# yisol/IDM-VTON

Measured on AMD Instinct MI355X. Metric: try-on images/sec at 768x1024, 30 DDIM steps, guidance 2.0, higher is better.
Workload: dtype bf16; 1 GPU; BASELINE.json configs[1]: 768x1024, 30 steps, batch 2/GPU, guidance 2.0, bf16 storage / fp32 accumulate, scheduler ddim, hipGraph on, GarmentNet batched over 6 timesteps, GarmentNet(block b+1)||TryonNet(block b) two-stream overlap on; images_per_call=2, parallelism=dp1 (image shards, one start-up RCCL weight broadcast), rccl_ranks=1

## Files before the change

### idm-vton_amd/csrc/attention.hip

```cpp
#include "common.cuh"

struct AttnParams {
    int B, heads, Nq;
    const void* q; int ldq; uint32_t qbytes;
    void* out; int ldo;
    int nseg;
    const void* k[2]; int ldk[2]; uint32_t kbytes[2];
    const void* vt[2]; int ldvt[2]; uint32_t vtbytes[2];
    int nk[2]; int krows[2]; int seg_b0[2];
    float ip_scale;
    int nqb, chunk, parts;
    int pp_flags; float pp_thr;
    int q_prescaled;
    int seg_nb[2];
    const int32_t* seg_ix[2];
    const int32_t* seg_nkt[2];
};

#define NEG_BIG (-1.0e30f)


__device__ __forceinline__ bool attn_work(const AttnParams& p, int bid, int& b, int& h, int& qb) {
    const int x = bid & 7, j = bid >> 3;
    const int u = j / p.chunk, r = j - u * p.chunk;
// ... 727 lines not shown
#pragma unroll
            for (int r = 0; r < 16; ++r) {
                const float pv = __builtin_amdgcn_exp2f(sacc[kb][r]);
                if constexpr (!LSUM) { if (r & 1) ps1 += pv; else ps0 += pv; }
                pf[kb * 2 + (r >> 3)][r & 7] = (T)pv;
            }
        if constexpr (!LSUM) l_run += ps0 + ps1;
        __builtin_amdgcn_sched_barrier(0);
        DBG_STAMP(5);
        const float nm = -m_run;
#pragma unroll
        for (int r = 0; r < 16; ++r) { sacc[0][r] = nm; sacc[1][r] = nm; }
        __builtin_amdgcn_sched_barrier(0);
        DBG_STAMP(6);
    };
    auto phase_barrier = [&]() {
        __builtin_amdgcn_sched_barrier(0);
        __builtin_amdgcn_s_barrier();
        __builtin_amdgcn_sched_barrier(0);
        asm volatile("" ::: "memory");
    };
    auto mid_barrier = [&](int s) {
        __builtin_amdgcn_sched_barrier(0);
        if (s + 2 <= sf.nt) asm volatile("s_waitcnt vmcnt(%0) lgkmcnt(0)" ::"n"(IPW) : "memory");
        else asm volatile("s_waitcnt vmcnt(0) lgkmcnt(0)" ::: "memory");
        __builtin_amdgcn_s_barrier();
        __builtin_amdgcn_sched_barrier(0);
        asm volatile("" ::: "memory");
    };
    int b0i = 0, b1i = 1;
    auto rotate = [&]() { b0i = b1i; b1i = b1i + 1 == ST ? 0 : b1i + 1; };

#ifdef ATTN_DBG
    dbg_t = __builtin_readcyclecounter();
#endif
    if (grp == 0) {
        read_frags(smem);
        for (int s = 0; s <= sf.nt; ++s) {
            asm volatile("s_waitcnt lgkmcnt(0)" ::: "memory");
            DBG_STAMP(2);
            phase_barrier();
            DBG_STAMP(3);
            mfma_block();
            __builtin_amdgcn_sched_barrier(0);
            DBG_STAMP(0);
            mid_barrier(s);
            DBG_STAMP(1);
            if ((ABL != 2 && ABL < 5) && s + 1 <= sf.nt) read_frags(smem + b1i * 16384);
            __builtin_amdgcn_sched_barrier(0);
            if ((ABL != 1 && ABL < 5) && s + 3 <= sf.nt) issue_stage(s + 3, b0i);
            if (s < sf.nt) valu_block(s);
            rotate();
        }
    } else {
        for (int s = 0; s <= sf.nt; ++s) {
            DBG_STAMP(2);
            phase_barrier();
            DBG_STAMP(3);
            if (ABL != 2 && ABL < 5) read_frags(smem + b0i * 16384);
            __builtin_amdgcn_sched_barrier(0);
            if (s >= 1) valu_block(s - 1);
            __builtin_amdgcn_sched_barrier(0);
            DBG_STAMP(0);
            mid_barrier(s);
            DBG_STAMP(1);
            mfma_block();
            __builtin_amdgcn_sched_barrier(0);
            if ((ABL != 1 && ABL < 5) && s + 3 <= sf.nt) issue_stage(s + 3, b0i);
            rotate();
        }
    }
#ifdef ATTN_DBG
    if (lane == 0 && blockIdx.x < 4096) {
#pragma unroll
        for (int i = 0; i < 8; ++i) g_attn_dbg[(blockIdx.x * 8 + wave) * 8 + i] = dbg_acc[i];
    }
#endif

    const float lt = LSUM ? lacc[0] : xhalf_sum(l_run);
    const float inv = lt > 0.f ? 1.0f / lt : 0.f;
    finalise_store<T>(p, b, h, q_row, u, oacc, inv);
}

template <typename T, int NW, int ABL = 0>
__global__ __launch_bounds__(NW * 64, 2) void attn_sp_kernel(const AttnParams p) {
    typedef typename VT<T>::v8 v8;
    constexpr int QB = 32 * NW, IPW = 16 / NW, ST = 3;
    __shared__ __attribute__((aligned(1024))) char smem[ST * 16384 + NW * 4096];

    const int lane = threadIdx.x & 63;
    const int wave = uniform(threadIdx.x >> 6);
    const int u = lane >> 5, l31 = lane & 31;
    const float limit = p.pp_thr;

    int b, h, qb;
    if (!sp_work(p, blockIdx.x, b, h, qb)) return;
    const int q_row = qb * QB + wave * 32 + l31;

    stage_q_tile(make_rsrc(p.q, p.qbytes), p.Nq, p.ldq, smem + ST * 16384 + wave * 4096, b, h, qb * QB + wave * 32, lane);
    SegFacts sf;
    seg_facts(p, b, sf);

    const int lrow = lane >> 3, lslot = lane & 7;
    const bool is_k = wave < NW / 2;
    uint32_t rb[IPW];
    auto seg_base = [&](int sg) {
        const size_t bsg = (size_t)(sg ? sf.bsg1 : sf.bsg0);
#pragma unroll
        for (int i = 0; i < IPW; ++i) {
            const int R = ((wave * IPW + i) & 7) * 8 + lrow;
            const int c = lslot ^ ((R >> 1) & 7);
            rb[i] = is_k ? (uint32_t)(((bsg * p.krows[sg] + R) * p.ldk[sg] + h * 64 + c * 8) * 2)
                         : (uint32_t)(((bsg * p.heads * 64 + h * 64 + R) * p.ldvt[sg] + c * 8) * 2);
        }
    };
    auto lane_lim = [&](int i) {
        const int R = ((wave * IPW + i) & 7) * 8 + lrow;
        const int c = lslot ^ ((R >> 1) & 7);
        return is_k ? R : 16 * (c >> 1) + 4 * (c & 1);
    };
    const uint32_t tstep0 = is_k ? (uint32_t)(64 * p.ldk[0] * 2) : 128u, tstep1 = is_k ? (uint32_t)(64 * p.ldk[1] * 2) : 128u;
    const __amdgpu_buffer_rsrc_t rs0 = is_k ? make_rsrc(p.k[0], p.kbytes[0]) : make_rsrc(p.vt[0], p.vtbytes[0]);
    const __amdgpu_buffer_rsrc_t rs1 = is_k ? make_rsrc(p.k[1], p.kbytes[1]) : make_rsrc(p.vt[1], p.vtbytes[1]);
    int ld_t = is_k ? 0 : -2, ld_room = sf.nt0 > 0 ? sf.nk0 : sf.nk1;
    bool ld_seg1 = sf.nt0 == 0;
    uint32_t ld_off = 0;
    seg_base(ld_seg1 ? 1 : 0);
    auto issue_next = [&](int bufi) {
        char* dst = smem + bufi * 16384 + wave * (IPW * 1024);
        if (ld_t < 0 || ld_t >= sf.nt) {
#pragma unroll
            for (int i = 0; i < IPW; ++i) dma16(rs0, dst + i * 1024, OOB_SENTINEL);
        } else {
            if (!ld_seg1 && ld_t == sf.nt0) { ld_seg1 = true; ld_off = 0; ld_room = sf.nk1; seg_base(1); }
            if (ld_room >= 64) {
#pragma unroll
                for (int i = 0; i < IPW; ++i) { if (ld_seg1) dma16(rs1, dst + i * 1024, rb[i] + ld_off); else dma16(rs0, dst + i * 1024, rb[i] + ld_off); }
            } else {
#pragma unroll
                for (int i = 0; i < IPW; ++i) {
                    const uint32_t off = lane_lim(i) < ld_room ? rb[i] + ld_off : OOB_SENTINEL;
                    if (ld_seg1) dma16(rs1, dst + i * 1024, off); else dma16(rs0, dst + i * 1024, off);
                }
            }
            ld_off += ld_seg1 ? tstep1 : tstep0;
            ld_room -= 64;
        }
        ++ld_t;
    };

    int f_addr[2], f_swz[2];
#pragma unroll
    for (int kb = 0; kb < 2; ++kb) { const int r = kb * 32 + l31; f_addr[kb] = r * 128; f_swz[kb] = (r >> 1) & 7; }

    f32x16 oacc[2], sA[2], sB[2];
    v8 P[4];
#pragma unroll
    for (int db = 0; db < 2; ++db)
#pragma unroll
        for (int r = 0; r < 16; ++r) { oacc[db][r] = 0.f; sA[db][r] = 0.f; sB[db][r] = 0.f; }
#pragma unroll
    for (int ks = 0; ks < 4; ++ks)
#pragma unroll
        for (int j = 0; j < 8; ++j) P[ks][j] = (T)0.f;
    float m_run = 0.f, l_run = 0.f;
    float lim_cur = -1.f, floor_cur = -3.0e38f;
    {
        const int nz = absent_keys(p, sf);
        if (nz > 0) { l_run = u == 0 ? (float)nz : 0.f; lim_cur = limit; floor_cur = 0.f; }
    }

    const int last = sf.nt + 1;
    issue_next(0);
    issue_next(1);
    wait_vmcnt<IPW>();
    __builtin_amdgcn_s_barrier();
    __builtin_amdgcn_sched_barrier(0);
    asm volatile("" ::: "memory");
    const char* const dq = smem + ST * 16384 + wave * 4096 + l31 * 128;
    v8 qf[4];
#pragma unroll
    for (int s4 = 0; s4 < 4; ++s4) qf[s4] = *(const v8*)(dq + (((2 * s4 + u) ^ ((l31 >> 1) & 7)) << 4));

    auto k_frag = [&](const char* buf, int kb, int s4) { return *(const v8*)(buf + f_addr[kb] + (((2 * s4 + u) ^ f_swz[kb]) << 4)); };
    auto v_frag = [&](const char* buf, int db, int ks) { return *(const v8*)(buf + 8192 + f_addr[db] + (((2 * ks + u) ^ f_swz[db]) << 4)); };

    int cbuf = 0, ibuf = 2;
    auto sync_stage = [&](int i) -> const char* {
        if (i + 1 <= last) wait_vmcnt<IPW>(); else wait_vmcnt<0>();
        if constexpr (!(ABL & 16)) __builtin_amdgcn_s_barrier();
        __builtin_amdgcn_sched_barrier(0);
        asm volatile("" ::: "memory");
        if (!(ABL & 8) && i + 2 <= last) issue_next(ibuf);
        const char* buf = smem + cbuf * 16384;
        cbuf = cbuf + 1 == ST ? 0 : cbuf + 1;
        ibuf = ibuf + 1 == ST ? 0 : ibuf + 1;
        return buf;
    };

    auto block = [&](int jvalid, const char* buf, f32x16 (&Scur)[2], f32x16 (&Snext)[2], float (&ps)[4]) {
        if (jvalid < 64) {
#pragma unroll
            for (int kb = 0; kb < 2; ++kb)
#pragma unroll
                for (int r = 0; r < 16; ++r) {
                    const int key = kb * 32 + (r & 3) + 8 * (r >> 2) + 4 * u;
                    if (key >= jvalid) Scur[kb][r] = NEG_BIG;
                }
        }
        __builtin_amdgcn_sched_barrier(0);
        v8 vf[2][4], kf[2][4];
#pragma unroll
        for (int ks = 0; ks < 4; ++ks) {
            if constexpr (ABL & 4) { vf[0][ks] = qf[ks]; vf[1][ks] = qf[ks]; kf[0][ks] = qf[ks]; kf[1][ks] = qf[ks]; }
            else { vf[0][ks] = v_frag(buf, 0, ks); vf[1][ks] = v_frag(buf, 1, ks); kf[0][ks] = k_frag(buf, 0, ks); kf[1][ks] = k_frag(buf, 1, ks); }
        }
        if constexpr (!(ABL & 2)) {
#pragma unroll
            for (int ks = 0; ks < 4; ++ks) {
                oacc[0] = VT<T>::mfma(vf[0][ks], P[ks], oacc[0]);
                oacc[1] = VT<T>::mfma(vf[1][ks], P[ks], oacc[1]);
                Snext[0] = VT<T>::mfma(kf[0][ks], qf[ks], Snext[0]);
                Snext[1] = VT<T>::mfma(kf[1][ks], qf[ks], Snext[1]);
            }
        } else {
#pragma unroll
            for (int ks = 0; ks < 4; ++ks) asm volatile("" :: "v"(vf[0][ks]), "v"(vf[1][ks]), "v"(kf[0][ks]), "v"(kf[1][ks]), "v"(P[ks]));
        }
        ps[0] = ps[1] = ps[2] = ps[3] = 0.f;
#pragma unroll
        for (int kb = 0; kb < 2; ++kb)
#pragma unroll
            for (int r = 0; r < 16; ++r) {
                const float pv = (ABL & 1) ? Scur[kb][r] : __builtin_amdgcn_exp2f(Scur[kb][r]);
                ps[r & 3] += pv;
                P[kb * 2 + (r >> 3)][r & 7] = (T)pv;
            }
#pragma unroll
        for (int ks = 0; ks < 4; ++ks) asm volatile("" : "+v"(P[ks]));
        __builtin_amdgcn_sched_barrier(0);
    };
    auto tail = [&](f32x16 (&Scur)[2], f32x16 (&Snext)[2], float (&ps)[4]) {
        float psum = (ps[0] + ps[1]) + (ps[2] + ps[3]);
        if (__any(!(psum <= lim_cur))) {
            float mx = fmaxf(Scur[0][0], Scur[1][0]);
#pragma unroll
            for (int r = 1; r < 16; ++r) mx = fmaxf(fmaxf(mx, Scur[0][r]), Scur[1][r]);
            mx = xhalf_max(mx);
            const float delta = fmaxf(mx, floor_cur);
            const float alpha = __builtin_amdgcn_exp2f(fminf(-delta, 0.f));
            l_run *= alpha;
#pragma unroll
            for (int db = 0; db < 2; ++db)
#pragma unroll
                for (int r = 0; r < 16; ++r) oacc[db][r] *= alpha;
            m_run += delta;
            lim_cur = limit; floor_cur = 0.f;
            float q0 = 0.f, q1 = 0.f;
#pragma unroll
            for (int kb = 0; kb < 2; ++kb)
#pragma unroll
                for (int r = 0; r < 16; ++r) {
                    const float pv = __builtin_amdgcn_exp2f(Scur[kb][r] - delta);
                    if (r & 1) q1 += pv; else q0 += pv;
                    P[kb * 2 + (r >> 3)][r & 7] = (T)pv;
                    Snext[kb][r] -= delta;
                }
            psum = q0 + q1;
        }
        l_run += psum;
        const float nm = -m_run;
#pragma unroll
        for (int r = 0; r < 16; ++r) { Scur[0][r] = nm; Scur[1][r] = nm; }
        __builtin_amdgcn_sched_barrier(0);
    };

    {
        const char* buf = sync_stage(0);
#pragma unroll
        for (int ks = 0; ks < 4; ++ks) {
            sA[0] = VT<T>::mfma(k_frag(buf, 0, ks), qf[ks], sA[0]);
            sA[1] = VT<T>::mfma(k_frag(buf, 1, ks), qf[ks], sA[1]);
        }
        __builtin_amdgcn_sched_barrier(0);
    }
    float ps[4];
    int i = 1, jv = sf.nt0 > 0 ? sf.nk0 : sf.nk1;
    auto next_valid = [&](int ii) { jv -= 64; if (ii == sf.nt0 && sf.nt1 > 0) jv = sf.nk1; };
    for (; i + 1 <= sf.nt; i += 2) {
        const char* buf = sync_stage(i);
        block(jv, buf, sA, sB, ps);
        tail(sA, sB, ps);
        next_valid(i);
        buf = sync_stage(i + 1);
        block(jv, buf, sB, sA, ps);
        tail(sB, sA, ps);
        next_valid(i + 1);
    }
    if (i <= sf.nt) {
        const char* buf = sync_stage(i);
        block(jv, buf, sA, sB, ps);
        tail(sA, sB, ps);
    }
    if (sf.nt > 0) {
        const char* buf = sync_stage(sf.nt + 1);
#pragma unroll
        for (int ks = 0; ks < 4; ++ks) {
            oacc[0] = VT<T>::mfma(v_frag(buf, 0, ks), P[ks], oacc[0]);
            oacc[1] = VT<T>::mfma(v_frag(buf, 1, ks), P[ks], oacc[1]);
        }
    }
    const float lt = xhalf_sum(l_run);
    const float inv = lt > 0.f ? 1.0f / lt : 0.f;
    finalise_store<T>(p, b, h, q_row, u, oacc, inv);
}

template <typename T, int MODE>
static int launch_attn(AttnParams& p, int tune, hipStream_t st) {
    const long bh = (long)p.B * p.heads;
    int nw = 4, stg = 3;
    if (bh * ((p.Nq + 255) / 256) >= 200) { nw = 8; stg = 2; }
    else if (bh * ((p.Nq + 127) / 128) < 64 && p.Nq <= 64) { nw = 2; stg = 2; }
    if (tune) { nw = tune & 0xff; stg = (tune >> 8) & 0xff; }
    else if (MODE == IDMVTON_ATTN_SELF && p.q_prescaled && p.Nq >= 128) {
        nw = (bh * ((p.Nq + 255) / 256) >= 400 && p.Nq >= 2048) ? 8 : 4; stg = 3;
        tune = (16 << 16) | (3 << 8) | nw;
    } else if (MODE == IDMVTON_ATTN_SELF && bh * ((p.Nq + 255) / 256) >= 200 && p.Nq >= 1024) {
        tune = (2 << 16) | (2 << 8) | 8; nw = 8; stg = 2;
    }
    const int kern = (tune >> 16) & 0xff, flags = (tune >> 24) & 3, sel = (tune >> 26) & 3;
    static const float thr_tab[4] = {4.f, 0.f, 8.f, 2.f};
    typedef void (*kernel_t)(const AttnParams);
    auto launch = [&](kernel_t k, bool sp, int qrows) -> int {
        dim3 grid;
        if (sp) sp_grid(p, qrows, grid); else attn_grid(p, qrows, grid);
        hipLaunchKernelGGL(k, grid, dim3(qrows * 2), 0, st, p);
        CHECK_LAUNCH("attn_fwd");
        return IDMVTON_OK;
    };
    if (kern == 2 || kern == 3) {
        const bool deep = kern == 3 && p.q_prescaled;
        if (MODE != IDMVTON_ATTN_SELF || nw != 8 || (stg != 2 && stg != 3))
            return idmvton_set_error(IDMVTON_E_ARG, "attn_fwd: the ping-pong kernel needs SELF mode, 8 waves, 2 or 3 stages");
        p.pp_flags = flags;
        p.pp_thr = thr_tab[sel];
        return launch(!deep ? attn_pp_kernel<T, 2, false> : stg == 2 ? attn_pp_kernel<T, 2, true> : attn_pp_kernel<T, 3, true>, false, 256);
    }
    if (kern >= 4 && kern <= 6) {
        p.pp_flags = 0; p.pp_thr = 4.f;
        if (MODE != IDMVTON_ATTN_SELF) return idmvton_set_error(IDMVTON_E_ARG, "attn_fwd: ablation kernels are SELF mode only");
        if (nw != 8 || stg != 2)
            return idmvton_set_error(IDMVTON_E_ARG, "attn_fwd: the ablation kernels are 8 waves, 2 stages (tune waves=%d stages=%d)", nw, stg);
        return launch(kern == 4 ? attn_pp_kernel<T, 2, false, 1> : kern == 5 ? attn_pp_kernel<T, 2, false, 2> : attn_pp_kernel<T, 2, false, 3>, false, 256);
    }
    if (kern == 7 || kern == 8) {
        if (MODE != IDMVTON_ATTN_SELF || !p.q_prescaled)
            return idmvton_set_error(IDMVTON_E_ARG, "attn_fwd: the prefetch kernel needs SELF mode and a pre-multiplied q");
        if (nw != 8 || stg != 3)
            return idmvton_set_error(IDMVTON_E_ARG, "attn_fwd: the prefetch kernel is 8 waves, 3 stages (tune waves=%d stages=%d)", nw, stg);
        p.pp_flags = 0;
        p.pp_thr = thr_tab[sel];
        return launch(kern == 7 ? attn_pf_kernel<T, true> : attn_pf_kernel<T, false>, false, 256);
    }
    if (kern == 16) {
        if (MODE != IDMVTON_ATTN_SELF || !p.q_prescaled)
            return idmvton_set_error(IDMVTON_E_ARG, "attn_fwd: the software-pipelined kernel needs SELF mode and a pre-multiplied q");
        if ((nw != 4 && nw != 8) || stg != 3)
            return idmvton_set_error(IDMVTON_E_ARG, "attn_fwd: the software-pipelined kernel is 4 or 8 waves, 3 stages (tune waves=%d stages=%d)", nw, stg);
        static const float lim_tab[4] = {512.f, 32.f, 8192.f, 128.f};
        p.pp_thr = lim_tab[sel];
        return nw == 4 ? launch(attn_sp_kernel<T, 4>, true, 128) : launch(attn_sp_kernel<T, 8>, true, 256);
    }
#ifdef ATTN_DBG
    if (kern >= 32 && kern < 160) {
        p.pp_flags = 0; p.pp_thr = 512.f;
        switch (kern - 32) {
#define SPA(m) case m: return launch(attn_sp_kernel<T, 8, m>, true, 256);
        SPA(0) SPA(1) SPA(2) SPA(3) SPA(4) SPA(8) SPA(12) SPA(15) SPA(16) SPA(31) SPA(29)
#undef SPA
        default: return idmvton_set_error(IDMVTON_E_ARG, "attn_fwd: ablation mask not built");
        }
    }
    if (kern >= 9 && kern <= 14) {
        p.pp_flags = 0; p.pp_thr = 4.f;
        switch (kern) {
        case 9: return launch(attn_pf_kernel<T, true, 1>, false, 256);
        case 10: return launch(attn_pf_kernel<T, true, 2>, false, 256);
        case 11: return launch(attn_pf_kernel<T, true, 3>, false, 256);
        case 12: return launch(attn_pf_kernel<T, true, 4>, false, 256);
        case 13: return launch(attn_pf_kernel<T, true, 5>, false, 256);
        default: return launch(attn_pf_kernel<T, true, 6>, false, 256);
        }
    }
#endif
    if (kern) return idmvton_set_error(IDMVTON_E_ARG, "attn_fwd: unknown kernel selector in tune");
    kernel_t k = nullptr;
#define ATTN_CASE(NW_, ST_) if (nw == NW_ && stg == ST_) k = attn_kernel<T, MODE, NW_, ST_>;
    ATTN_CASE(2, 2) ATTN_CASE(4, 2) ATTN_CASE(8, 2)
    ATTN_CASE(2, 3) ATTN_CASE(4, 3) ATTN_CASE(8, 3)
    ATTN_CASE(2, 4) ATTN_CASE(4, 4) ATTN_CASE(8, 4)
#undef ATTN_CASE
    if (!k) return idmvton_set_error(IDMVTON_E_ARG, "attn_fwd: unsupported tune (waves=%d stages=%d)", nw, stg);
    return launch(k, false, 32 * nw);
}

static int attn_fwd_impl(const idmvton_attn_args* a, const int32_t* seg_nb, const int32_t* const* seg_index, const int32_t* const* seg_nk, void* stream) {
    CHECK_ARG(a != nullptr, IDMVTON_E_ARG, "attn_fwd: null args");
    CHECK_ARG(a->dtype == IDMVTON_F16 || a->dtype == IDMVTON_BF16, IDMVTON_E_DTYPE, "attn_fwd: dtype %d", a->dtype);
    CHECK_ARG(a->mode == IDMVTON_ATTN_SELF || a->mode == IDMVTON_ATTN_CROSS, IDMVTON_E_ARG, "attn_fwd: mode %d", a->mode);
    CHECK_ARG(a->B > 0 && a->heads > 0 && a->Nq > 0, IDMVTON_E_SHAPE, "attn_fwd: B=%d heads=%d Nq=%d", a->B, a->heads, a->Nq);
    CHECK_ARG(a->nseg >= 1 && a->nseg <= 2, IDMVTON_E_SHAPE, "attn_fwd: nseg=%d", a->nseg);
    if (a->mode == IDMVTON_ATTN_CROSS) CHECK_ARG(a->nseg == 2 && a->seg_b0[0] == 0 && a->seg_b0[1] == 0, IDMVTON_E_ARG,
                                                 "attn_fwd: CROSS needs two segments present for every batch");
    CHECK_ARG(a->q && a->out && a->ldq % 8 == 0 && a->ldo % 8 == 0 && ((uintptr_t)a->q & 15) == 0 && ((uintptr_t)a->out & 15) == 0,
              IDMVTON_E_ALIGN, "attn_fwd: q/out alignment (ldq=%d ldo=%d)", a->ldq, a->ldo);
    CHECK_ARG(a->ldq >= a->heads * 64 && a->ldo >= a->heads * 64, IDMVTON_E_SHAPE, "attn_fwd: ldq/ldo < heads*64");
    AttnParams p;
    p.B = a->B; p.heads = a->heads; p.Nq = a->Nq; p.q = a->q; p.ldq = a->ldq; p.out = a->out; p.ldo = a->ldo;
    p.nseg = a->nseg; p.ip_scale = a->ip_scale; p.nqb = 0; p.chunk = p.parts = 1; p.pp_flags = 0; p.pp_thr = 4.f; p.q_prescaled = a->q_prescaled ? 1 : 0;
    const uint64_t qb = ((uint64_t)a->B * a->Nq - 1) * a->ldq * 2 + (uint64_t)a->heads * 128;
    CHECK_ARG(qb < 0x80000000ull, IDMVTON_E_SHAPE, "attn_fwd: Q >= 2 GiB");
    p.qbytes = (uint32_t)qb;
    for (int s = 0; s < 2; ++s) {
        const int ss = s < a->nseg ? s : 0;
        CHECK_ARG(a->k[ss] && a->vt[ss] && a->nk[ss] > 0 && a->seg_b0[ss] >= 0 && a->seg_b0[ss] <= a->B,
                  IDMVTON_E_SHAPE, "attn_fwd: seg %d nk=%d b0=%d", ss, a->nk[ss], a->seg_b0[ss]);
        const int32_t* ix = seg_index ? seg_index[ss] : nullptr;
        if (ix) {
            CHECK_ARG(a->mode != IDMVTON_ATTN_CROSS, IDMVTON_E_ARG, "attn_fwd_indexed: CROSS mode takes no table (seg %d)", ss);
            CHECK_ARG(seg_nb[ss] >= 1 && a->seg_b0[ss] < a->B, IDMVTON_E_SHAPE,
                      "attn_fwd_indexed: seg %d has a table: needs seg_nb >= 1 (%d) and seg_b0 < B (%d, %d)", ss, seg_nb[ss], a->seg_b0[ss], a->B);
            CHECK_ARG(((uintptr_t)ix & 3) == 0, IDMVTON_E_ALIGN, "attn_fwd_indexed: seg %d table is not 4-byte aligned", ss);
        } else
        CHECK_ARG(seg_nb[ss] >= 0 && seg_nb[ss] <= a->B - a->seg_b0[ss], IDMVTON_E_SHAPE,
                  "attn_fwd_shared: seg %d seg_nb=%d outside [0, B - seg_b0 = %d]", ss, seg_nb[ss], a->B - a->seg_b0[ss]);
        const int32_t* nkt = seg_nk && s < a->nseg ? seg_nk[s] : nullptr;
        if (nkt) {
            CHECK_ARG(a->mode != IDMVTON_ATTN_CROSS, IDMVTON_E_ARG, "attn_fwd_ragged: CROSS mode takes no table (seg %d)", ss);
            CHECK_ARG(((uintptr_t)nkt & 3) == 0, IDMVTON_E_ALIGN, "attn_fwd_ragged: seg %d key-count table is not 4-byte aligned", ss);
        }
        CHECK_ARG(a->mode != IDMVTON_ATTN_CROSS || seg_nb[ss] == 0, IDMVTON_E_ARG, "attn_fwd_shared: CROSS mode takes seg_nb = {0, 0} (seg %d: %d)", ss, seg_nb[ss]);
        const int krows = a->k_rows[ss] > 0 ? a->k_rows[ss] : a->nk[ss];
        CHECK_ARG(krows >= a->nk[ss], IDMVTON_E_SHAPE, "attn_fwd: seg %d k_rows=%d < nk", ss, krows);
        CHECK_ARG(a->ldk[ss] % 8 == 0 && a->ldvt[ss] % 16 == 0 && a->ldvt[ss] >= ((a->nk[ss] + 15) & ~15) && a->ldk[ss] >= a->heads * 64 &&
                  ((uintptr_t)a->k[ss] & 15) == 0 && ((uintptr_t)a->vt[ss] & 15) == 0, IDMVTON_E_ALIGN,
                  "attn_fwd: seg %d ldk=%d ldvt=%d (V^T is read in key order: ldvt %% 16 == 0, ldvt >= roundup16(nk))", ss, a->ldk[ss], a->ldvt[ss]);
        const int nb = seg_nb[ss] > 0 ? seg_nb[ss] : a->B - a->seg_b0[ss];
        const uint64_t kb = (uint64_t)nb * krows * a->ldk[ss] * 2, vb = (uint64_t)nb * a->heads * 64 * a->ldvt[ss] * 2;
        CHECK_ARG(kb < 0x80000000ull && vb < 0x80000000ull, IDMVTON_E_SHAPE, "attn_fwd: seg %d K/V^T >= 2 GiB", ss);
        p.k[s] = a->k[ss]; p.ldk[s] = a->ldk[ss]; p.kbytes[s] = (uint32_t)kb;
        p.vt[s] = a->vt[ss]; p.ldvt[s] = a->ldvt[ss]; p.vtbytes[s] = (uint32_t)vb;
        p.nk[s] = a->nk[ss]; p.krows[s] = krows; p.seg_b0[s] = a->seg_b0[ss]; p.seg_nb[s] = seg_nb[ss]; p.seg_ix[s] = ix; p.seg_nkt[s] = nkt;
    }
    hipStream_t st = (hipStream_t)stream;
    if (a->dtype == IDMVTON_BF16)
        return a->mode == IDMVTON_ATTN_SELF ? launch_attn<bf16_t, IDMVTON_ATTN_SELF>(p, a->tune, st) : launch_attn<bf16_t, IDMVTON_ATTN_CROSS>(p, a->tune, st);
    return a->mode == IDMVTON_ATTN_SELF ? launch_attn<f16_t, IDMVTON_ATTN_SELF>(p, a->tune, st) : launch_attn<f16_t, IDMVTON_ATTN_CROSS>(p, a->tune, st);
}

extern "C" int idmvton_attn_fwd(const idmvton_attn_args* a, void* stream) {
    static const int32_t none[2] = {0, 0};
    return attn_fwd_impl(a, none, nullptr, nullptr, stream);
}

extern "C" int idmvton_attn_fwd_shared(const idmvton_attn_args* a, const int32_t seg_nb[2], void* stream) {
    CHECK_ARG(seg_nb != nullptr, IDMVTON_E_ARG, "attn_fwd_shared: null seg_nb");
    return attn_fwd_impl(a, seg_nb, nullptr, nullptr, stream);
}

extern "C" int idmvton_attn_fwd_indexed(const idmvton_attn_args* a, const int32_t seg_nb[2], const int32_t* const seg_index[2], void* stream) {
    CHECK_ARG(seg_nb != nullptr && seg_index != nullptr, IDMVTON_E_ARG, "attn_fwd_indexed: null seg_nb / seg_index");
    return attn_fwd_impl(a, seg_nb, seg_index, nullptr, stream);
}

extern "C" int idmvton_attn_fwd_ragged(const idmvton_attn_args* a, const int32_t seg_nb[2], const int32_t* const seg_index[2],
                                       const int32_t* const seg_nk[2], void* stream) {
    CHECK_ARG(seg_nb != nullptr && seg_nk != nullptr, IDMVTON_E_ARG, "attn_fwd_ragged: null seg_nb / seg_nk");
    return attn_fwd_impl(a, seg_nb, seg_index, seg_nk, stream);
}
```

### idm-vton_amd/ffi.py

```python
import ctypes as C
import functools
import os

_HERE = os.path.dirname(os.path.abspath(__file__))
LIB_PATH = os.environ.get("IDMVTON_HIP_LIB") or os.path.join(_HERE, "libidmvton_hip.so")

F16, BF16, F32, F8E4M3 = 0, 1, 2, 3
EPI_NONE, EPI_GEGLU, EPI_GELU, EPI_QUICKGELU, EPI_XATTN = 0, 1, 2, 3, 4
ATTN_SELF, ATTN_CROSS = 0, 1
IO_RES_F32, IO_OUT_F32, IO_BIAS_F32, IO_OUT_F8 = 1, 2, 4, 8
GN_X_F32, GN_Y_SPLIT, GN_AFFINE_F32 = 1, 2, 4
LAYOUT_SPLIT, LAYOUT_NHWC_F32 = 1, 2
SPLIT_ACT, SPLIT_W3, SPLIT_W3T = 0, 1, 2
KVS_WIDEN_E4M3, KVS_COPY = 0, 1
MAX_SEG = 24
ABI_VERSION = 9

i32, u32, f32, vp = C.c_int32, C.c_uint32, C.c_float, C.c_void_p


class Seg(C.Structure):
    _fields_ = [("ptr", vp), ("bytes", u32), ("pitch", i32), ("coff", i32), ("len", i32), ("dy", i32), ("dx", i32)]


# ... 28 lines not shown
                ("flags", i32)]


class PackInputArgs(C.Structure):
    _fields_ = [("dtype", i32), ("B", i32), ("hw", i32), ("cpad", i32), ("latents", vp), ("cond", vp), ("out", vp)]


class CfgStepArgs(C.Structure):
    _fields_ = [("dtype", i32), ("B", i32), ("hw", i32), ("ldc", i32), ("eps_nhwc", vp), ("latents", vp),
                ("noise", vp), ("coef", vp)]


class GuidedStepArgs(C.Structure):
    _fields_ = [("dtype", i32), ("B", i32), ("hw", i32), ("ldc", i32), ("branches", i32), ("work_floats", i32), ("eps_nhwc", vp),
                ("latents", vp), ("noise", vp), ("coef", vp), ("work", vp)]


class LayoutArgs(C.Structure):
    _fields_ = [("dtype", i32), ("B", i32), ("C", i32), ("HW", i32), ("cpad", i32), ("to_nhwc", i32), ("src", vp),
                ("dst", vp), ("scale", f32), ("shift", f32), ("flags", i32)]


class VaeSampleArgs(C.Structure):
    _fields_ = [("dtype", i32), ("B", i32), ("hw", i32), ("ldm", i32), ("moments", vp), ("noise", vp), ("z", vp),
                ("scale", f32)]


class AttnSmallArgs(C.Structure):
    _fields_ = [("dtype", i32), ("B", i32), ("heads", i32), ("Lq", i32), ("Lk", i32), ("d", i32), ("q", vp), ("ldq", i32),
                ("k", vp), ("ldk", i32), ("v", vp), ("ldv", i32), ("out", vp), ("ldo", i32), ("scale", f32), ("causal", i32)]


class AttnF8Args(C.Structure):
    _fields_ = [("out_dtype", i32), ("B", i32), ("heads", i32), ("Nq", i32), ("q8", vp), ("ldq", i32), ("out", vp), ("ldo", i32),
                ("nseg", i32), ("k8", vp * 2), ("ldk", i32 * 2), ("vt8", vp * 2), ("ldvt", i32 * 2), ("nk", i32 * 2), ("k_rows", i32 * 2),
                ("seg_b0", i32 * 2), ("qk_scale_exp", i32), ("v_scale_exp", i32)]


class QuantF8Args(C.Structure):
    _fields_ = [("dtype", i32), ("mode", i32), ("rows", i32), ("cols", i32), ("src", vp), ("lds", i32), ("dst", vp), ("ldd", i32), ("scale", f32)]


class SoftmaxArgs(C.Structure):
    _fields_ = [("dtype", i32), ("rows", i32), ("n", i32), ("ld", i32), ("x", vp), ("scale", f32), ("y_split", vp), ("ldy", i32), ("n_valid", i32)]


class SplitArgs(C.Structure):
    _fields_ = [("dtype", i32), ("mode", i32), ("rows", i32), ("cols", i32), ("src", vp), ("lds", i32), ("dst", vp), ("ldd", i32)]


class KvUnpackDesc(C.Structure):
    _fields_ = [("src", vp), ("dst", vp), ("exp", vp), ("rows", i32), ("cols", i32), ("lds", i32), ("ldd", i32)]


class KvUnpackArgs(C.Structure):
    _fields_ = [("dtype", i32), ("n", i32), ("desc", vp), ("max_chunks", i32)]


class KvStreamDesc(KvUnpackDesc):
    pass


class KvStreamArgs(C.Structure):
    _fields_ = [("dtype", i32), ("mode", i32), ("n", i32), ("workgroups", i32), ("desc", vp), ("first", vp)]


STRUCTS = {"idmvton_seg": Seg, "idmvton_gemm_conv_args": GemmConvArgs, "idmvton_attn_args": AttnArgs,
           "idmvton_layernorm_args": LayerNormArgs, "idmvton_groupnorm_args": GroupNormArgs,
           "idmvton_pack_input_args": PackInputArgs, "idmvton_cfg_step_args": CfgStepArgs,
           "idmvton_layout_args": LayoutArgs, "idmvton_vae_sample_args": VaeSampleArgs, "idmvton_softmax_args": SoftmaxArgs,
           "idmvton_attn_small_args": AttnSmallArgs, "idmvton_attn_f8_args": AttnF8Args, "idmvton_quant_f8_args": QuantF8Args,
           "idmvton_split_args": SplitArgs, "idmvton_xattn": XAttn, "idmvton_kv_unpack_desc": KvUnpackDesc,
           "idmvton_kv_unpack_args": KvUnpackArgs, "idmvton_kv_stream_desc": KvStreamDesc, "idmvton_kv_stream_args": KvStreamArgs,
           "idmvton_guided_step_args": GuidedStepArgs}

SYMBOLS = ["idmvton_last_error", "idmvton_abi_version", "idmvton_sizeof", "idmvton_gemm_conv", "idmvton_attn_fwd",
           "idmvton_layernorm", "idmvton_groupnorm", "idmvton_pack_input", "idmvton_cfg_step", "idmvton_layout",
           "idmvton_vae_sample", "idmvton_softmax_rows", "idmvton_probe_mfma", "idmvton_groupnorm_stats_doubles",
           "idmvton_attn_small", "idmvton_rccl_unique_id", "idmvton_rccl_comm_init", "idmvton_rccl_bcast_arena",
           "idmvton_rccl_comm_destroy", "idmvton_attn_f8", "idmvton_quant_f8", "idmvton_split", "idmvton_attn_fwd_shared",
           "idmvton_attn_f8_shared", "idmvton_attn_fwd_indexed", "idmvton_attn_f8_indexed",
           "idmvton_attn_fwd_ragged", "idmvton_attn_f8_ragged", "idmvton_kv_unpack", "idmvton_kv_stream",
           "idmvton_host_device_ptr", "idmvton_kv_fill", "idmvton_kv_place", "idmvton_guided_step", "idmvton_guided_step_work_floats",
           "idmvton_pack_input_cond"]

_lib = None


class HipLibraryMissing(RuntimeError):
    pass


def lib():
    global _lib
    if _lib is not None:
        return _lib
    if not os.path.exists(LIB_PATH):
        raise HipLibraryMissing(f"{LIB_PATH} not built: run `make -C {os.path.join(_HERE, 'csrc')}` "
                                "(or __graft_entry__.build()); there is no CPU fallback")
    L = C.CDLL(LIB_PATH)
    for s in SYMBOLS:
        if not hasattr(L, s):
            raise HipLibraryMissing(f"{LIB_PATH} does not export {s}")
    L.idmvton_last_error.restype = C.c_char_p
    L.idmvton_sizeof.argtypes = [C.c_char_p]
    L.idmvton_abi_version.restype = C.c_int
    v = L.idmvton_abi_version()
    if v != ABI_VERSION:
        raise HipLibraryMissing(f"{LIB_PATH} implements C ABI version {v}, this binding needs {ABI_VERSION}: rebuild it "
                                f"(`make -C {os.path.join(_HERE, 'csrc')}`)")
    for name, st in STRUCTS.items():
        n = L.idmvton_sizeof(name.encode())
        if n != C.sizeof(st):
            raise HipLibraryMissing(f"ABI drift: sizeof({name}) is {n} in the library, {C.sizeof(st)} in ffi.py")
    for s in ("idmvton_gemm_conv", "idmvton_attn_fwd", "idmvton_layernorm", "idmvton_groupnorm",
              "idmvton_pack_input", "idmvton_cfg_step", "idmvton_layout", "idmvton_vae_sample", "idmvton_softmax_rows",
              "idmvton_attn_small", "idmvton_attn_f8", "idmvton_quant_f8", "idmvton_split", "idmvton_guided_step", "idmvton_pack_input_cond"):
        getattr(L, s).argtypes = [vp, vp]
        getattr(L, s).restype = C.c_int
    for s in ("idmvton_attn_fwd_shared", "idmvton_attn_f8_shared"):
        getattr(L, s).argtypes = [vp, C.POINTER(i32), vp]
        getattr(L, s).restype = C.c_int
    for s in ("idmvton_attn_fwd_indexed", "idmvton_attn_f8_indexed"):
        getattr(L, s).argtypes = [vp, C.POINTER(i32), C.POINTER(vp), vp]
        getattr(L, s).restype = C.c_int
    for s in ("idmvton_attn_fwd_ragged", "idmvton_attn_f8_ragged"):
        getattr(L, s).argtypes = [vp, C.POINTER(i32), C.POINTER(vp), C.POINTER(vp), vp]
        getattr(L, s).restype = C.c_int
    L.idmvton_kv_unpack.argtypes = [vp, vp, vp]
    L.idmvton_kv_unpack.restype = C.c_int
    for s in ("idmvton_kv_stream", "idmvton_kv_fill", "idmvton_kv_place"):
        getattr(L, s).argtypes = [vp, vp, vp, vp]
        getattr(L, s).restype = C.c_int
    L.idmvton_host_device_ptr.argtypes = [vp, C.POINTER(vp)]
    L.idmvton_host_device_ptr.restype = C.c_int
    L.idmvton_probe_mfma.argtypes = [C.c_int, vp, vp, vp, vp]
    L.idmvton_groupnorm_stats_doubles.argtypes = [C.c_int] * 4
    L.idmvton_groupnorm_stats_doubles.restype = C.c_int
    L.idmvton_guided_step_work_floats.argtypes = [C.c_int] * 2
    L.idmvton_guided_step_work_floats.restype = C.c_int
    L.idmvton_rccl_unique_id.argtypes = [vp]
    L.idmvton_rccl_comm_init.argtypes = [vp, C.c_int, C.c_int, C.POINTER(vp)]
    L.idmvton_rccl_bcast_arena.argtypes = [vp, vp, C.c_uint64, C.c_int, C.c_uint64, vp]
    L.idmvton_rccl_comm_destroy.argtypes = [vp]
    for s in ("idmvton_rccl_unique_id", "idmvton_rccl_comm_init", "idmvton_rccl_bcast_arena", "idmvton_rccl_comm_destroy"):
        getattr(L, s).restype = C.c_int
    _lib = L
    return L


def call(fn_name, args, stream):
    L = lib()
    rc = getattr(L, fn_name)(C.byref(args), C.c_void_p(stream))
    if rc != 0:
        raise RuntimeError(f"{fn_name} failed ({rc}): {L.idmvton_last_error().decode()}")


def call_shared(fn_name, args, seg_nb, stream):
    L = lib()
    nb = (i32 * 2)(*seg_nb)
    rc = getattr(L, fn_name)(C.byref(args), nb, C.c_void_p(stream))
    if rc != 0:
        raise RuntimeError(f"{fn_name} failed ({rc}): {L.idmvton_last_error().decode()}")


def call_indexed(fn_name, args, seg_nb, seg_index, stream):
    L = lib()
    nb = (i32 * 2)(*seg_nb)
    ix = (vp * 2)(*[int(x) if x else None for x in seg_index])
    rc = getattr(L, fn_name)(C.byref(args), nb, ix, C.c_void_p(stream))
    if rc != 0:
        raise RuntimeError(f"{fn_name} failed ({rc}): {L.idmvton_last_error().decode()}")


def call_ragged(fn_name, args, seg_nb, seg_index, seg_nk, stream):
    L = lib()
    nb = (i32 * 2)(*seg_nb)
    ix = (vp * 2)(*[int(x) if x else None for x in (seg_index or (0, 0))])
    nk = (vp * 2)(*[int(x) if x else None for x in seg_nk])
    rc = getattr(L, fn_name)(C.byref(args), nb, ix, nk, C.c_void_p(stream))
    if rc != 0:
        raise RuntimeError(f"{fn_name} failed ({rc}): {L.idmvton_last_error().decode()}")


def call_kv_unpack(args, host_desc, stream):
    L = lib()
    rc = L.idmvton_kv_unpack(C.byref(args), host_desc if isinstance(host_desc, int) else C.cast(host_desc, vp), C.c_void_p(stream))
    if rc != 0:
        raise RuntimeError(f"idmvton_kv_unpack failed ({rc}): {L.idmvton_last_error().decode()}")


def _call_kv_table(fn_name, args, host_desc, host_first, stream):
    L = lib()
    p = lambda x: x if isinstance(x, int) else C.cast(x, vp)
    rc = getattr(L, fn_name)(C.byref(args), p(host_desc), p(host_first), C.c_void_p(stream))
    if rc != 0:
        raise RuntimeError(f"{fn_name} failed ({rc}): {L.idmvton_last_error().decode()}")


call_kv_stream = functools.partial(_call_kv_table, "idmvton_kv_stream")
call_kv_fill = functools.partial(_call_kv_table, "idmvton_kv_fill")
call_kv_place = functools.partial(_call_kv_table, "idmvton_kv_place")


def host_device_ptr(host):
    L = lib()
    dev = vp()
    rc = L.idmvton_host_device_ptr(C.c_void_p(host), C.byref(dev))
    if rc != 0:
        raise RuntimeError(f"idmvton_host_device_ptr failed ({rc}): {L.idmvton_last_error().decode()}")
    return int(dev.value)
```

### include/idmvton_hip.h

```cpp
#ifndef IDMVTON_HIP_H
#define IDMVTON_HIP_H
#include <stddef.h>
#include <stdint.h>

#ifdef __cplusplus
extern "C" {
#endif

enum { IDMVTON_OK = 0, IDMVTON_E_SHAPE = -1, IDMVTON_E_DTYPE = -2, IDMVTON_E_ALIGN = -3, IDMVTON_E_LAUNCH = -4,
       IDMVTON_E_ARG = -5 };
enum { IDMVTON_F16 = 0, IDMVTON_BF16 = 1, IDMVTON_F32 = 2, IDMVTON_F8E4M3 = 3  };

const char* idmvton_last_error(void);
int idmvton_abi_version(void);
int idmvton_sizeof(const char* struct_name);

#define IDMVTON_MAX_SEG 24
typedef struct {
    const void* ptr;
    uint32_t bytes;
    int32_t pitch;
    int32_t coff;
    int32_t len;
    int32_t dy, dx;
} idmvton_seg;

enum { IDMVTON_EPI_NONE = 0, IDMVTON_EPI_GEGLU = 1, IDMVTON_EPI_GELU = 2 ,
       IDMVTON_EPI_QUICKGELU = 3 ,
       IDMVTON_EPI_XATTN = 4  };
typedef struct {
    int32_t nseg;
    const void* k[2]; int32_t ldk[2]; int32_t k_rows[2];
    const void* vt[2]; int32_t ldvt[2];
    int32_t nk[2];
    int32_t tokens; float ip_scale;
} idmvton_xattn;
enum { IDMVTON_IO_RES_F32 = 1, IDMVTON_IO_OUT_F32 = 2, IDMVTON_IO_BIAS_F32 = 4, IDMVTON_IO_OUT_F8 = 8 };
typedef struct {
    int32_t dtype;
    const void* w; int32_t N; int32_t Ktot;
    int32_t nseg; idmvton_seg seg[IDMVTON_MAX_SEG];
    int32_t M, Ho, Wo, Hi, Wi, stride, ups;
    void* out; int32_t ldo;
    const void* bias;
    const void* rowbias; int32_t rowbias_ld; int32_t rows_per_group;
    const void* res; int32_t ldr;
    int32_t mode;
    void* vt; int32_t vt_n0; int32_t vt_tokens;
    int32_t tile_hint;
    int32_t vt_perm;
    int32_t io_flags;
    const idmvton_xattn* xattn;
    int32_t colscale_n; float colscale;
    float f8_out_scale, f8_vt_scale;
} idmvton_gemm_conv_args;
int idmvton_gemm_conv(const idmvton_gemm_conv_args* a, void* stream);

enum { IDMVTON_ATTN_SELF = 0, IDMVTON_ATTN_CROSS = 1 };
typedef struct {
    int32_t dtype; int32_t mode;
    int32_t B, heads, Nq;
    const void* q; int32_t ldq;
    void* out; int32_t ldo;
    int32_t nseg;
    const void* k[2]; int32_t ldk[2];
    const void* vt[2]; int32_t ldvt[2];
    int32_t nk[2];
    int32_t k_rows[2];
    int32_t seg_b0[2];
    float ip_scale;
    int32_t tune;
    int32_t q_prescaled;
} idmvton_attn_args;
int idmvton_attn_fwd(const idmvton_attn_args* a, void* stream);
int idmvton_attn_fwd_shared(const idmvton_attn_args* a, const int32_t seg_nb[2], void* stream);
int idmvton_attn_fwd_indexed(const idmvton_attn_args* a, const int32_t seg_nb[2], const int32_t* const seg_index[2], void* stream);
int idmvton_attn_fwd_ragged(const idmvton_attn_args* a, const int32_t seg_nb[2], const int32_t* const seg_index[2],
                            const int32_t* const seg_nk[2], void* stream);

typedef struct {
    int32_t out_dtype; int32_t B, heads, Nq;
    const void* q8; int32_t ldq;
    void* out; int32_t ldo;
    int32_t nseg;
    const void* k8[2]; int32_t ldk[2];
    const void* vt8[2]; int32_t ldvt[2];
    int32_t nk[2]; int32_t k_rows[2]; int32_t seg_b0[2];
    int32_t qk_scale_exp; int32_t v_scale_exp;
} idmvton_attn_f8_args;
int idmvton_attn_f8(const idmvton_attn_f8_args* a, void* stream);
int idmvton_attn_f8_shared(const idmvton_attn_f8_args* a, const int32_t seg_nb[2], void* stream);
int idmvton_attn_f8_indexed(const idmvton_attn_f8_args* a, const int32_t seg_nb[2], const int32_t* const seg_index[2], void* stream);
int idmvton_attn_f8_ragged(const idmvton_attn_f8_args* a, const int32_t seg_nb[2], const int32_t* const seg_index[2],
                           const int32_t* const seg_nk[2], void* stream);
typedef struct {
    int32_t dtype; int32_t mode; int32_t rows, cols;
    const void* src; int32_t lds;
    void* dst; int32_t ldd;
    float scale;
} idmvton_quant_f8_args;
int idmvton_quant_f8(const idmvton_quant_f8_args* a, void* stream);

typedef struct {
    const void* src;
    void* dst;
    const int32_t* exp;
    int32_t rows, cols, lds, ldd;
} idmvton_kv_unpack_desc;
typedef struct {
    int32_t dtype; int32_t n;
    const idmvton_kv_unpack_desc* desc;
    int32_t max_chunks;
} idmvton_kv_unpack_args;
int idmvton_kv_unpack(const idmvton_kv_unpack_args* a, const idmvton_kv_unpack_desc* host_desc, void* stream);

enum { IDMVTON_KVS_WIDEN_E4M3 = 0, IDMVTON_KVS_COPY = 1 };
#define IDMVTON_KVS_MAX_N (1 << 20)
typedef idmvton_kv_unpack_desc idmvton_kv_stream_desc;
typedef struct {
    int32_t dtype; int32_t mode; int32_t n; int32_t workgroups;
    const idmvton_kv_stream_desc* desc;
    const int32_t* first;
} idmvton_kv_stream_args;
int idmvton_kv_stream(const idmvton_kv_stream_args* a, const idmvton_kv_stream_desc* host_desc, const int32_t* host_first, void* stream);
int idmvton_host_device_ptr(const void* host, void** dev);

int idmvton_kv_fill(const idmvton_kv_stream_args* a, const idmvton_kv_stream_desc* host_desc, const int32_t* host_first, void* stream);

int idmvton_kv_place(const idmvton_kv_stream_args* a, const idmvton_kv_stream_desc* host_desc, const int32_t* host_first, void* stream);

typedef struct {
    int32_t dtype; int32_t B, heads, Lq, Lk, d;
    const void* q; int32_t ldq;
    const void* k; int32_t ldk;
    const void* v; int32_t ldv;
    void* out; int32_t ldo;
    float scale; int32_t causal;
} idmvton_attn_small_args;
int idmvton_attn_small(const idmvton_attn_small_args* a, void* stream);

typedef struct {
    int32_t dtype; int32_t rows, C;
    const void* x; int32_t ldx;
    const void* gamma; const void* beta; float eps;
    void* y; int32_t ldy;
    void* y2; int32_t ldy2;
    int32_t x_f32;
} idmvton_layernorm_args;
int idmvton_layernorm(const idmvton_layernorm_args* a, void* stream);

enum { IDMVTON_GN_X_F32 = 1 , IDMVTON_GN_Y_SPLIT = 2 ,
       IDMVTON_GN_AFFINE_F32 = 4  };
typedef struct {
    int32_t dtype; int32_t B, HW, C, groups;
    const void* x; int32_t C1;
    const void* x2;
    const void* gamma; const void* beta; float eps; int32_t silu;
    void* y;
    double* stats; int32_t stats_doubles;
    int32_t flags;
} idmvton_groupnorm_args;
// ... 67 lines not shown
```

Before: 1.631 images/s.

## Add unrolled fast path for full key tiles in pipelined self-attention kernel

Adds a fast path to the software-pipelined self-attention kernel. Runs of full 64-key tiles that do not touch a partial tile or the segment edge are processed in unrolled groups of six, with stage buffer indices fixed at compile time, no key masking and no partial-tile bounds checks on loads. Segment switching is simplified to a single precomputed tile index with a current resource descriptor, and out-of-range loads now use a zero-size descriptor. It also adds a FAST=false variant (kern 31) for comparison and a host helper that counts fast groups, at the cost of larger code and more logic to get right at group boundaries.

```diff
diff --git a/idm-vton_amd/csrc/attention.hip b/idm-vton_amd/csrc/attention.hip
--- a/idm-vton_amd/csrc/attention.hip
+++ b/idm-vton_amd/csrc/attention.hip
@@ -833,7 +833,19 @@
     finalise_store<T>(p, b, h, q_row, u, oacc, inv);
 }
 
-template <typename T, int NW, int ABL = 0>
+__host__ __device__ inline bool sp_group_ok(int i, int nt0, int nt1, int nk0, int nk1) {
+    const int nt = nt0 + nt1;
+    if (i + 7 > nt - 1) return false;
+    const int part0 = (nt0 > 0 && (nk0 & 63)) ? nt0 - 1 : -1;
+    const int part1 = (nt1 > 0 && (nk1 & 63)) ? nt - 1 : -1;
+    return !(part0 >= i - 1 && part0 <= i + 7) && !(part1 >= i - 1 && part1 <= i + 7);
+}
+__host__ __device__ inline int sp_fast_groups(int nt0, int nt1, int nk0, int nk1) {
+    int n = 0;
+    for (int i = 3; sp_group_ok(i, nt0, nt1, nk0, nk1); i += 6) ++n;
+    return n;
+}
+template <typename T, int NW, int ABL = 0, bool FAST = true>
 __global__ __launch_bounds__(NW * 64, 2) void attn_sp_kernel(const AttnParams p) {
     typedef typename VT<T>::v8 v8;
     constexpr int QB = 32 * NW, IPW = 16 / NW, ST = 3;
@@ -852,11 +864,13 @@
     SegFacts sf;
     seg_facts(p, b, sf);
 
-    const int lrow = lane >> 3, lslot = lane & 7;
     const bool is_k = wave < NW / 2;
     uint32_t rb[IPW];
     auto seg_base = [&](int sg) {
         const size_t bsg = (size_t)(sg ? sf.bsg1 : sf.bsg0);
+        int ln = lane;
+        asm volatile("" : "+v"(ln));
+        const int lrow = ln >> 3, lslot = ln & 7;
 #pragma unroll
         for (int i = 0; i < IPW; ++i) {
             const int R = ((wave * IPW + i) & 7) * 8 + lrow;
@@ -866,6 +880,9 @@
         }
     };
     auto lane_lim = [&](int i) {
+        int ln = lane;
+        asm volatile("" : "+v"(ln));
+        const int lrow = ln >> 3, lslot = ln & 7;
         const int R = ((wave * IPW + i) & 7) * 8 + lrow;
         const int c = lslot ^ ((R >> 1) & 7);
         return is_k ? R : 16 * (c >> 1) + 4 * (c & 1);
@@ -873,30 +890,39 @@
     const uint32_t tstep0 = is_k ? (uint32_t)(64 * p.ldk[0] * 2) : 128u, tstep1 = is_k ? (uint32_t)(64 * p.ldk[1] * 2) : 128u;
     const __amdgpu_buffer_rsrc_t rs0 = is_k ? make_rsrc(p.k[0], p.kbytes[0]) : make_rsrc(p.vt[0], p.vtbytes[0]);
     const __amdgpu_buffer_rsrc_t rs1 = is_k ? make_rsrc(p.k[1], p.kbytes[1]) : make_rsrc(p.vt[1], p.vtbytes[1]);
+    const __amdgpu_buffer_rsrc_t rs_zero = make_rsrc(is_k ? p.k[0] : p.vt[0], 0);
     int ld_t = is_k ? 0 : -2, ld_room = sf.nt0 > 0 ? sf.nk0 : sf.nk1;
-    bool ld_seg1 = sf.nt0 == 0;
+    int ld_sw = sf.nt0 > 0 && sf.nt1 > 0 ? sf.nt0 : -3;
+    __amdgpu_buffer_rsrc_t rs_cur = sf.nt0 > 0 ? rs0 : rs1;
+    uint32_t tstep_cur = sf.nt0 > 0 ? tstep0 : tstep1;
     uint32_t ld_off = 0;
-    seg_base(ld_seg1 ? 1 : 0);
+    seg_base(sf.nt0 > 0 ? 0 : 1);
+    auto switch_seg = [&]() { ld_sw = -3; rs_cur = rs1; tstep_cur = tstep1; ld_off = 0; ld_room = sf.nk1; seg_base(1); };
     auto issue_next = [&](int bufi) {
         char* dst = smem + bufi * 16384 + wave * (IPW * 1024);
         if (ld_t < 0 || ld_t >= sf.nt) {
 #pragma unroll
-            for (int i = 0; i < IPW; ++i) dma16(rs0, dst + i * 1024, OOB_SENTINEL);
+            for (int i = 0; i < IPW; ++i) dma16(rs_zero, dst + i * 1024, rb[i]);
         } else {
-            if (!ld_seg1 && ld_t == sf.nt0) { ld_seg1 = true; ld_off = 0; ld_room = sf.nk1; seg_base(1); }
+            if (ld_t == ld_sw) switch_seg();
             if (ld_room >= 64) {
 #pragma unroll
-                for (int i = 0; i < IPW; ++i) { if (ld_seg1) dma16(rs1, dst + i * 1024, rb[i] + ld_off); else dma16(rs0, dst + i * 1024, rb[i] + ld_off); }
+                for (int i = 0; i < IPW; ++i) dma16(rs_cur, dst + i * 1024, rb[i] + ld_off);
             } else {
 #pragma unroll
-                for (int i = 0; i < IPW; ++i) {
-                    const uint32_t off = lane_lim(i) < ld_room ? rb[i] + ld_off : OOB_SENTINEL;
-                    if (ld_seg1) dma16(rs1, dst + i * 1024, off); else dma16(rs0, dst + i * 1024, off);
-                }
-            }
-            ld_off += ld_seg1 ? tstep1 : tstep0;
+                for (int i = 0; i < IPW; ++i) dma16(rs_cur, dst + i * 1024, lane_lim(i) < ld_room ? rb[i] + ld_off : OOB_SENTINEL);
+            }
+            ld_off += tstep_cur;
             ld_room -= 64;
         }
+        ++ld_t;
+    };
+    auto issue_full = [&](char* dst) {
+        if (ld_t == ld_sw) switch_seg();
+#pragma unroll
+        for (int i = 0; i < IPW; ++i) dma16(rs_cur, dst + i * 1024, rb[i] + ld_off);
+        ld_off += tstep_cur;
+        ld_room -= 64;
         ++ld_t;
     };
 
@@ -949,17 +975,21 @@
         return buf;
     };
 
-    auto block = [&](int jvalid, const char* buf, f32x16 (&Scur)[2], f32x16 (&Snext)[2], float (&ps)[4]) {
+    auto mask_keys = [&](int jvalid, f32x16 (&Scur)[2]) {
         if (jvalid < 64) {
+            int u4 = 4 * u;
+            asm volatile("" : "+v"(u4));
 #pragma unroll
             for (int kb = 0; kb < 2; ++kb)
 #pragma unroll
                 for (int r = 0; r < 16; ++r) {
-                    const int key = kb * 32 + (r & 3) + 8 * (r >> 2) + 4 * u;
+                    const int key = kb * 32 + (r & 3) + 8 * (r >> 2) + u4;
                     if (key >= jvalid) Scur[kb][r] = NEG_BIG;
                 }
         }
         __builtin_amdgcn_sched_barrier(0);
+    };
+    auto block = [&](const char* buf, f32x16 (&Scur)[2], f32x16 (&Snext)[2], float (&ps)[4]) {
         v8 vf[2][4], kf[2][4];
 #pragma unroll
         for (int ks = 0; ks < 4; ++ks) {
@@ -1038,19 +1068,47 @@
     float ps[4];
     int i = 1, jv = sf.nt0 > 0 ? sf.nk0 : sf.nk1;
     auto next_valid = [&](int ii) { jv -= 64; if (ii == sf.nt0 && sf.nt1 > 0) jv = sf.nk1; };
+    auto group_iter = [&](auto kc, f32x16 (&Scur)[2], f32x16 (&Snext)[2]) {
+        constexpr int k = decltype(kc)::value;
+        wait_vmcnt<IPW>();
+        if constexpr (!(ABL & 16)) __builtin_amdgcn_s_barrier();
+        __builtin_amdgcn_sched_barrier(0);
+        asm volatile("" ::: "memory");
+        if constexpr (!(ABL & 8)) issue_full(smem + ((2 + k) % 3) * 16384 + wave * (IPW * 1024));
+        __builtin_amdgcn_sched_barrier(0);
+        block(smem + (k % 3) * 16384, Scur, Snext, ps);
+        tail(Scur, Snext, ps);
+    };
+    auto general_iter = [&](int ii, f32x16 (&Scur)[2], f32x16 (&Snext)[2]) {
+        const char* buf = sync_stage(ii);
+        mask_keys(jv, Scur);
+        block(buf, Scur, Snext, ps);
+        tail(Scur, Snext, ps);
+        next_valid(ii);
+    };
+    if (FAST && sp_group_ok(3, sf.nt0, sf.nt1, sf.nk0, sf.nk1)) {
+        general_iter(1, sA, sB);
+        general_iter(2, sB, sA);
+        i = 3;
+        do {
+            group_iter(std::integral_constant<int, 0>(), sA, sB);
+            group_iter(std::integral_constant<int, 1>(), sB, sA);
+            group_iter(std::integral_constant<int, 2>(), sA, sB);
+            group_iter(std::integral_constant<int, 3>(), sB, sA);
+            group_iter(std::integral_constant<int, 4>(), sA, sB);
+            group_iter(std::integral_constant<int, 5>(), sB, sA);
+            i += 6;
+        } while (sp_group_ok(i, sf.nt0, sf.nt1, sf.nk0, sf.nk1));
+        jv = i - 1 < sf.nt0 ? sf.nk0 - (i - 1) * 64 : sf.nk1 - (i - 1 - sf.nt0) * 64;
+    }
     for (; i + 1 <= sf.nt; i += 2) {
-        const char* buf = sync_stage(i);
-        block(jv, buf, sA, sB, ps);
-        tail(sA, sB, ps);
-        next_valid(i);
-        buf = sync_stage(i + 1);
-        block(jv, buf, sB, sA, ps);
-        tail(sB, sA, ps);
-        next_valid(i + 1);
+        general_iter(i, sA, sB);
+        general_iter(i + 1, sB, sA);
     }
     if (i <= sf.nt) {
         const char* buf = sync_stage(i);
-        block(jv, buf, sA, sB, ps);
+        mask_keys(jv, sA);
+        block(buf, sA, sB, ps);
         tail(sA, sB, ps);
     }
     if (sf.nt > 0) {
@@ -1113,13 +1171,14 @@
         p.pp_thr = thr_tab[sel];
         return launch(kern == 7 ? attn_pf_kernel<T, true> : attn_pf_kernel<T, false>, false, 256);
     }
-    if (kern == 16) {
+    if (kern == 16 || kern == 31) {
         if (MODE != IDMVTON_ATTN_SELF || !p.q_prescaled)
             return idmvton_set_error(IDMVTON_E_ARG, "attn_fwd: the software-pipelined kernel needs SELF mode and a pre-multiplied q");
         if ((nw != 4 && nw != 8) || stg != 3)
             return idmvton_set_error(IDMVTON_E_ARG, "attn_fwd: the software-pipelined kernel is 4 or 8 waves, 3 stages (tune waves=%d stages=%d)", nw, stg);
         static const float lim_tab[4] = {512.f, 32.f, 8192.f, 128.f};
         p.pp_thr = lim_tab[sel];
+        if (kern == 31) return nw == 4 ? launch(attn_sp_kernel<T, 4, 0, false>, true, 128) : launch(attn_sp_kernel<T, 8, 0, false>, true, 256);
         return nw == 4 ? launch(attn_sp_kernel<T, 4>, true, 128) : launch(attn_sp_kernel<T, 8>, true, 256);
     }
 #ifdef ATTN_DBG
@@ -1209,6 +1268,8 @@
     return a->mode == IDMVTON_ATTN_SELF ? launch_attn<f16_t, IDMVTON_ATTN_SELF>(p, a->tune, st) : launch_attn<f16_t, IDMVTON_ATTN_CROSS>(p, a->tune, st);
 }
 
+extern "C" int idmvton_attn_sp_fast_groups(int nt0, int nt1, int nk0, int nk1) { return sp_fast_groups(nt0, nt1, nk0, nk1); }
+
 extern "C" int idmvton_attn_fwd(const idmvton_attn_args* a, void* stream) {
     static const int32_t none[2] = {0, 0};
     return attn_fwd_impl(a, none, nullptr, nullptr, stream);
diff --git a/idm-vton_amd/ffi.py b/idm-vton_amd/ffi.py
--- a/idm-vton_amd/ffi.py
+++ b/idm-vton_amd/ffi.py
@@ -134,7 +134,7 @@
            "idmvton_attn_f8_shared", "idmvton_attn_fwd_indexed", "idmvton_attn_f8_indexed",
            "idmvton_attn_fwd_ragged", "idmvton_attn_f8_ragged", "idmvton_kv_unpack", "idmvton_kv_stream",
            "idmvton_host_device_ptr", "idmvton_kv_fill", "idmvton_kv_place", "idmvton_guided_step", "idmvton_guided_step_work_floats",
-           "idmvton_pack_input_cond"]
+           "idmvton_pack_input_cond", "idmvton_attn_sp_fast_groups"]
 
 _lib = None
 
@@ -191,6 +191,8 @@
     L.idmvton_groupnorm_stats_doubles.restype = C.c_int
     L.idmvton_guided_step_work_floats.argtypes = [C.c_int] * 2
     L.idmvton_guided_step_work_floats.restype = C.c_int
+    L.idmvton_attn_sp_fast_groups.argtypes = [C.c_int] * 4
+    L.idmvton_attn_sp_fast_groups.restype = C.c_int
     L.idmvton_rccl_unique_id.argtypes = [vp]
     L.idmvton_rccl_comm_init.argtypes = [vp, C.c_int, C.c_int, C.POINTER(vp)]
     L.idmvton_rccl_bcast_arena.argtypes = [vp, vp, C.c_uint64, C.c_int, C.c_uint64, vp]
diff --git a/include/idmvton_hip.h b/include/idmvton_hip.h
--- a/include/idmvton_hip.h
+++ b/include/idmvton_hip.h
@@ -77,6 +77,7 @@
 int idmvton_attn_fwd_indexed(const idmvton_attn_args* a, const int32_t seg_nb[2], const int32_t* const seg_index[2], void* stream);
 int idmvton_attn_fwd_ragged(const idmvton_attn_args* a, const int32_t seg_nb[2], const int32_t* const seg_index[2],
                             const int32_t* const seg_nk[2], void* stream);
+int idmvton_attn_sp_fast_groups(int nt0, int nt1, int nk0, int nk1);
 
 typedef struct {
     int32_t out_dtype; int32_t B, heads, Nq;
```

Result: no change. 1.638 images/s (median of 6 runs) (+0.4%).
